# arielnetworks/tidal-wave

Hardware: AMD Instinct MI355X
Metric: image-pairs/sec @1080p Farneback (default params), 1/2/4/8 MI355X (higher is better)
Workload: dtype f32

## Files before the change

### tidal-wave_amd/csrc/twflow.hip

```cpp
#include "twflow_kernels.hip.h"

#include <hip/hip_runtime.h>
#include <unistd.h>

#include <dlfcn.h>
#include <float.h>
#include <math.h>
#include <stdio.h>
#include <stdlib.h>
#include <string.h>

#include <chrono>
#include <map>
#include <mutex>
#include <string>
#include <tuple>
#include <utility>
#include <vector>

#include "../../include/twflow.h"
#include "../../include/twflow_debug.h"

using namespace twk;

// ... 398 lines not shown
    int upd_ny = 2;
    int scan_fused = 0;
    int poly_f32 = 0;
    long long mfree_min_px = 0;
    int mfree_min_w = 320;
    int mfree = 1;
    int cu_count = 256;
    int pyr23_threads = 0;
    int blur_cm = 0;
    int pyr_fused = 1;
    int pyr_generic = 0;
    int blur_variant = 4;
    int pp_waves = 512;
    unsigned long long* dbg_stamps = nullptr;
    int blur_nomask = 0;
    int blur_pipe = 0;
    int blur_small = -1;
    int blur_small_lv[8] = {-1, -1, -1, -1, -1, -1, -1, -1};
    int poly_variant = 1;
    std::string err;
    size_t ws_elems = 0;
    float *I = nullptr, *R = nullptr, *M[2] = {nullptr, nullptr};
    std::vector<float*> flow;
    std::vector<size_t> flow_cap;
    int lat_streams = 1;
    long long lat_min_px = 100000;
    float *lat_I = nullptr, *lat_R = nullptr;
    size_t lat_cap = 0;
    std::vector<hipEvent_t> lat_ev;
    int lat_s2_max = 1000;
    int ramp = 1;
    int fi_maxseg = 4, fi_minsteps = 16;
    int fi_skip = 0;
    int fi_nt = 1024;
    int lat_fused = 1;
    int lat_graph = 0;
    std::map<GraphKey, hipGraphExec_t> lat_graphs;
    hipStream_t copy_stream = nullptr;
    hipStream_t d2h_stream = nullptr;
    long long d2h_ops = 0;
    int d2h_sync_skipped = 0;
    FlowDst* d_fdst = nullptr;
    FlowDst* d_fsrc = nullptr;
    const uint8_t** d_ptrs = nullptr;
    int* d_count = nullptr;
    float2* d_grid = nullptr;
    size_t d_grid_cap = 0;
    int prof_level[TW_K_COUNT] = {-2, -2, -2, -2, -2};
    std::vector<ProfPair> prof_pending[TW_K_COUNT];
    std::vector<hipEvent_t> prof_free;
    unsigned long long launches[TW_DF_COUNT] = {};
    unsigned long long last_grid_z[TW_DF_COUNT] = {};
};

namespace {

#define TW_LAUNCH(e, fam, kern, grid, ...)                         \
    do {                                                           \
        const dim3 _g = (grid);                                    \
        if (e) {                                                   \
            (e)->launches[fam]++;                                  \
            (e)->last_grid_z[fam] = _g.z;                          \
        }                                                          \
        hipLaunchKernelGGL(kern, _g, __VA_ARGS__);                 \
    } while (0)

#define TW_HIP(e, call)                                                                   \
// ... 635 lines not shown
    return pl->levels >= 1 && pl->lv[0].ksize == 3 && pl->lv[1].ksize == 3 && pl->lv[0].mode == 0 && pl->lv[1].mode == 2 &&
           pl->w0 == 2 * pl->lv[1].w && pl->h0 == 2 * pl->lv[1].h && pl->w0 >= 16;
}
void launch_pyr01(tw_engine* e, hipStream_t st, const Plan* pl, const uint8_t* const* d_srcs, long long stride, float* I1,
                  float* I0, int nimg)
{
    const LevelPlan &L0 = pl->lv[0], &L1 = pl->lv[1];
    PyrK3fArgs a;
    a.srcs = d_srcs;
    a.dst0 = I0;
    a.dst1 = I1;
    a.zs0 = L0.ps;
    a.zs1 = L1.ps;
    a.stride = stride;
    a.w0 = pl->w0;
    a.h0 = pl->h0;
    a.ld0 = L0.ld;
    a.w1 = L1.w;
    a.h1 = L1.h;
    a.ld1 = L1.ld;
    a.a0 = L0.h_kern[1];
    a.a1 = L0.h_kern[0];
    a.b0 = L1.h_kern[1];
    a.b1 = L1.h_kern[0];
    a.aligned4 = (stride % 4 == 0) ? e->img_aligned4 : 0;
    ProfScope ps(e, st, TW_K_PYR, 1);
    TW_LAUNCH(e, TW_DF_PYR_K3F, tw_pyr_k3f, dim3((L1.w + 255) / 256, (L1.h + 3) / 4, nimg), dim3(256), 0, st, a);
}

bool flow_iter_eligible(const tw_engine* e, int w, int h)
{
    return e->win_m == 15 && !e->box && w >= e->mfree_min_w && h >= 4 * FI_TH;
}
bool level_runs_flow_iter(const tw_engine* e, int w, int h, int nc, bool lat, bool grid_only)
{
    const int it = e->p.pyrIterations;
    const int fi_out = (e->fi_nt == 512 ? FI_SC_512 : FI_SC) - 30;
    const long long fi_wgs = (long long)((w + fi_out - 1) / fi_out) * std::min(4, std::max(1, h / (16 * FI_TH))) * nc;
    return e->mfree && !lat && it > (grid_only ? 1 : 0) && flow_iter_eligible(e, w, h) &&
           (fi_wgs * 4 >= (long long)e->cu_count * 3 || e->mfree == 2) &&
           (e->mfree_min_px <= 0 || (long long)w * h >= e->mfree_min_px);
}
bool single_pair_schedule(const tw_engine* e, int n, int w0, int h0, int levels)
{
    return n == 1 && e->lat_streams && levels >= 1 && (long long)w0 * h0 >= e->lat_min_px;
}
bool scan_fused_level0(const tw_engine* e, int span)
{
    return e->p.pyrIterations > 0 && e->scan_fused && span == 10 && e->win_m == 15 && !e->box;
}
int balanced_launch_pairs(int n, int chunk)
{
    const int nlaunch = (n + chunk - 1) / chunk;
    return nlaunch > 0 ? (n + nlaunch - 1) / nlaunch : 1;
}
struct FlowUps {
    const float* prev;
    int pw, ph, pld;
    long long pfps;
    const int *xofs, *yofs;
    const float *alpha, *beta;
    int xmax;
    float scale;
};
void launch_flow_iter(tw_engine* e, hipStream_t st, int w, int h, int ld, long long ps, const float* R, const float* flow_in,
                      long long fps_in, float* flow_out, long long fps_out, const FlowUps* ups, int npairs, int level)
{
    FlowIterArgs a;
    memset(&a, 0, sizeof(a));
    a.R = R;
    a.flow_in = flow_in;
    a.flow_out = flow_out;
    a.w = w;
    a.h = h;
    a.ld = ld;
    a.ps = ps;
    a.fps_in = fps_in;
    a.fps_out = fps_out;
    a.zero_flow = (!flow_in && !ups) ? 1 : 0;
    a.c = e->wc;
#ifdef TW_VARIANTS
    a.dbg_skip = e->fi_skip;
    a.dbg = (unsigned long long*)e->dbg_stamps;
#endif
    const int OUT = (e->fi_nt == 512 ? FI_SC_512 : FI_SC) - 30;
    const int slots = e->cu_count * (e->fi_nt == 512 ? 2 : 1);
    const int nstrips = (w + OUT - 1) / OUT, nsteps = (h + FI_TH - 1) / FI_TH;
    int best_seg = 1;
    double best_cost = 1e300;
    for (int sg = 1; sg <= e->fi_maxseg; sg++) {
        const int nt = (nsteps + sg - 1) / sg;
        if (sg > 1 && nt < e->fi_minsteps) break;
        const long long wgs = (long long)nstrips * sg * npairs;
        const long long rounds = (wgs + slots - 1) / slots;
        const double cost = (double)rounds * (nt + 7 * 0.25);
        if (cost < best_cost) {
            best_cost = cost;
            best_seg = sg;
        }
    }
    a.nt = (nsteps + best_seg - 1) / best_seg;
    const int nseg = (nsteps + a.nt - 1) / a.nt;
    const dim3 grid(nstrips, nseg, npairs);
    ProfScope pscope(e, st, TW_K_BLUR_SOLVE, level);
    if (ups) {
        a.prev = ups->prev;
        a.pw = ups->pw;
        a.ph = ups->ph;
        a.pld = ups->pld;
        a.pfps = ups->pfps;
        a.xofs = ups->xofs;
        a.alpha = ups->alpha;
        a.yofs = ups->yofs;
        a.beta = ups->beta;
        a.xmax = ups->xmax;
        a.scale = ups->scale;
    }
#ifdef TW_VARIANTS
    if (e->fi_nt == 512) {
        if (ups) TW_LAUNCH(e, TW_DF_FLOW_ITER_UPS, (tw_flow_iter<15, 1, 512>), grid, dim3(512), 0, st, a);
        else if (a.zero_flow) TW_LAUNCH(e, TW_DF_FLOW_ITER_ZERO, (tw_flow_iter<15, 2, 512>), grid, dim3(512), 0, st, a);
        else TW_LAUNCH(e, TW_DF_FLOW_ITER, (tw_flow_iter<15, 0, 512>), grid, dim3(512), 0, st, a);
        return;
    }
#endif
    if (ups) {
        TW_LAUNCH(e, TW_DF_FLOW_ITER_UPS, (tw_flow_iter<15, 1>), grid, dim3(1024), 0, st, a);
    } else if (a.zero_flow) {
        TW_LAUNCH(e, TW_DF_FLOW_ITER_ZERO, (tw_flow_iter<15, 2>), grid, dim3(1024), 0, st, a);
    } else {
        TW_LAUNCH(e, TW_DF_FLOW_ITER, (tw_flow_iter<15, 0>), grid, dim3(1024), 0, st, a);
    }
}

struct GridOut {
    float2* g;
    int span, gw, gh;
    bool* used;
};
void launch_blur(tw_engine* e, hipStream_t st, int w, int h, int ld, long long ps, const float* Min, float* Mout,
                 float* flow, const float* R, int update, int level, int npairs, double* Vbox = nullptr,
                 const SideJob* side = nullptr, bool* side_used = nullptr, const GridOut* go = nullptr, bool quads = false)
{
    BlurArgs a;
    a.Min = Min;
    a.Mout = Mout;
    a.flow = flow;
    a.R = R;
    a.w = w;
    a.h = h;
    a.ld = ld;
    a.ps = ps;
    a.fps = ps;
    a.update = update;
    a.xsh = 0;
    a.rot = 0;
    a.store_flow = level < 0 ? 1 : 0;
    a.m = e->win_m;
// ... 1381 lines not shown
            e->blur_small_lv[k] = atoi(q);
            while (*q && *q != ',') q++;
            if (*q == ',') q++;
        }
    }
    if (const char* ev = getenv("TW_PP_WAVES")) e->pp_waves = atoi(ev);
    if (const char* ev = getenv("TW_BLUR_NOMASK")) e->blur_nomask = atoi(ev);
    if (const char* ev = getenv("TW_BLUR_PIPE")) e->blur_pipe = atoi(ev);
    if (const char* ev = getenv("TW_POLYEXP_F32")) e->poly_f32 = atoi(ev) == 2 ? 2 : (atoi(ev) ? 1 : 0);
#ifndef TW_VARIANTS
    {
        bool bad_lv = false;
        for (int v : e->blur_small_lv) bad_lv = bad_lv || v == 2 || v == 3 || v == 5;
        const bool bad = bad_lv || (e->blur_variant != 4) || (e->poly_variant != 1) || (e->blur_pipe != 0) || (e->blur_small == 2 || e->blur_small == 3 ||
                         e->blur_small == 5) || (getenv("TW_UPD_NY") && atoi(getenv("TW_UPD_NY")) == 1);
        if (bad) {
            fprintf(stderr, "twflow: TW_BLUR_VARIANT / TW_POLY_VARIANT / TW_BLUR_PIPE / TW_BLUR_SMALL=2,3,5 / TW_UPD_NY=1 select kernels "
                            "that are only in a VARIANTS=1 build (tidal-wave_amd/libtwflow_variants.so)\n");
            delete e;
            return TW_E_UNSUPPORTED;
        }
    }
#endif
    if (const char* ev = getenv("TW_DEBUG_STAMPS"))
        if (atoi(ev) && hipMalloc((void**)&e->dbg_stamps, 4096 * sizeof(unsigned long long)) == hipSuccess)
            (void)hipMemset(e->dbg_stamps, 0, 4096 * sizeof(unsigned long long));
    if (const char* ev = getenv("TW_UPD_NY")) e->upd_ny = atoi(ev) == 1 ? 1 : 2;
    if (const char* ev = getenv("TW_LANES")) e->lanes = std::min(2, std::max(1, atoi(ev)));
    if (const char* ev = getenv("TW_LATENCY_STREAMS")) e->lat_streams = atoi(ev) ? 1 : 0;
    if (const char* ev = getenv("TW_LATENCY_MIN_PX")) e->lat_min_px = atoll(ev);
    if (const char* ev = getenv("TW_LAT_GRAPH")) e->lat_graph = atoi(ev) ? 1 : 0;
    if (const char* ev = getenv("TW_LAT_FUSED")) e->lat_fused = atoi(ev) ? 1 : 0;
#ifdef TW_VARIANTS
    if (const char* ev = getenv("TW_FI_NT")) e->fi_nt = atoi(ev) == 512 ? 512 : 1024;
    if (const char* ev = getenv("TW_FI_SKIP")) e->fi_skip = atoi(ev);
#endif
    if (const char* ev = getenv("TW_LAT_S2_LEVELS")) e->lat_s2_max = atoi(ev);
    if (const char* ev = getenv("TW_RAMP")) e->ramp = atoi(ev) ? 1 : 0;
    if (const char* ev = getenv("TW_FI_MAXSEG")) e->fi_maxseg = std::min(64, std::max(1, atoi(ev)));
    if (const char* ev = getenv("TW_FI_MINSTEPS")) e->fi_minsteps = std::max(2, atoi(ev));
    int prio_lo = 0, prio_hi = 0;
    (void)hipDeviceGetStreamPriorityRange(&prio_lo, &prio_hi);
    bool ok = hipStreamCreateWithPriority(&e->stream, hipStreamNonBlocking, prio_hi) == hipSuccess &&
              hipStreamCreateWithPriority(&e->stream2, hipStreamNonBlocking, e->lanes > 1 ? prio_hi : prio_lo) == hipSuccess &&
              hipStreamCreateWithFlags(&e->copy_stream, hipStreamNonBlocking) == hipSuccess &&
              hipEventCreateWithFlags(&e->ev_fork, hipEventDisableTiming) == hipSuccess &&
              hipEventCreateWithFlags(&e->ev_join, hipEventDisableTiming) == hipSuccess &&
              hipMalloc((void**)&e->d_ptrs, sizeof(void*) * 2 * slots + 256) == hipSuccess &&
              hipMalloc((void**)&e->d_count, sizeof(int) * slots + 256) == hipSuccess;
    for (Ctx& c : e->ctx) {
        ok = ok && hipEventCreate(&c.ev_start) == hipSuccess && hipEventCreate(&c.ev_stop) == hipSuccess &&
             hipEventCreateWithFlags(&c.ev_done, hipEventDisableTiming) == hipSuccess &&
             hipEventCreateWithFlags(&c.ev_h2d, hipEventDisableTiming) == hipSuccess &&
             hipEventCreateWithFlags(&c.ev_seg[0], hipEventDisableTiming) == hipSuccess &&
             hipEventCreateWithFlags(&c.ev_seg[1], hipEventDisableTiming) == hipSuccess &&
             hipHostMalloc((void**)&c.h_ptrs, sizeof(void*) * 2 * slots, hipHostMallocDefault) == hipSuccess &&
             hipHostMalloc((void**)&c.h_count, sizeof(int) * slots, hipHostMallocDefault) == hipSuccess &&
             hipHostMalloc((void**)&c.h_png, sizeof(PngJob) * 2 * (size_t)slots, hipHostMallocDefault) == hipSuccess &&
             hipMalloc((void**)&c.d_png, sizeof(PngJob) * 2 * (size_t)slots + 256) == hipSuccess &&
             hipHostMalloc((void**)&c.h_rec, sizeof(ScanRec) * HOST_RECS * (size_t)slots, hipHostMallocDefault) ==
                 hipSuccess;
    }
    if (!ok) {
        tw_engine_destroy(e);
        return TW_E_DEVICE;
    }
    *out = e;
// ... 1135 lines not shown
```

### tidal-wave_amd/csrc/twflow_kernels.hip.h

```cpp
#pragma once
#include <hip/hip_runtime.h>
#include <stdint.h>
#include <type_traits>

namespace twk {

typedef float __attribute__((ext_vector_type(4))) f32x4;
typedef const float __attribute__((address_space(1))) * gptr_cf;
typedef const char __attribute__((address_space(1))) * gptr_cc;

__device__ __forceinline__ gptr_cf sgpr_base(const float* p)
{
    gptr_cf g = (gptr_cf)p;
    asm volatile("" : "+s"(g));
    return g;
}
__device__ __forceinline__ float gload(gptr_cf row, unsigned byte_off)
{
    return *(gptr_cf)((gptr_cc)row + byte_off);
}
typedef float __attribute__((address_space(1))) * gptr_f;
typedef char __attribute__((address_space(1))) * gptr_c;
__device__ __forceinline__ gptr_f sgpr_base_w(float* p)
{
// ... 1795 lines not shown
            bstore(rsF, ob, 0u, fxv);
            bstore(rsF, ob, (unsigned)(a.fps * 4), fyv);
            if (a.gspan > 0) {
                const unsigned qx = __umulhi((unsigned)xc, a.gmagic), qy = __umulhi((unsigned)yc, a.gmagic);
                if (qx * (unsigned)a.gspan == (unsigned)xc && qy * (unsigned)a.gspan == (unsigned)yc)
                    a.grid[((long long)z * a.gh + qy) * a.gw + qx] = float2{fxv, fyv};
            }
        }
        if (FUSED) {
            if (a.update) {
                float M[5];
                if constexpr (QPRE) update_matrices_core(qpre[i], R1, a.ps, a.ld, a.w, a.h, xc, yc, fxv, fyv, M);
                else update_matrices_px(R0, R1, a.ps, a.ld, a.w, a.h, xc, yc, fxv, fyv, M);
                if (valid) {
                    if constexpr ((TW_NT & 1) == 0) {
#pragma unroll
                        for (int cc = 0; cc < 5; cc++) bstore(rsM, ob, (unsigned)(cc * a.ps * 4), M[cc]);
                    } else {
#pragma unroll
                        for (int cc = 0; cc < 5; cc++) st_stream<0>(Mout + o + cc * a.ps, M[cc]);
                    }
                }
            }
        }
    }
}
template <int MH, int COLS, int HALO, int TH, bool FUSED, int VILP = 2, int HILP = 2, int SUNROLL = 2, bool QPRE = true, bool VPRE = true>
__global__ __launch_bounds__(COLS) __attribute__((amdgpu_waves_per_eu(4, 8))) void tw_blur_solve4(BlurArgs a)
{
    __shared__ __attribute__((aligned(16))) float sm[5][TH][COLS];
    tw_blur_solve4_body<MH, COLS, HALO, TH, FUSED, VILP, HILP, SUNROLL, QPRE, VPRE>(a, hw_grid(), hw_block(), sm);
}

constexpr int FI_TH = 5, FI_SC = 190, FI_PITCH = 192;
constexpr int FI_SC_512 = 94, FI_PITCH_512 = 96;
struct FlowIterArgs {
    const float* R;
    const float* flow_in;
    float* flow_out;
    int w, h, ld;
    long long ps, fps_in, fps_out;
    int nt;
    int zero_flow;
    const float* prev;
    int pw, ph, pld;
    long long pfps;
    const int* xofs;
    const float* alpha;
    const int* yofs;
    const float* beta;
    int xmax;
    float scale;
    unsigned long long* dbg;
    int dbg_skip;
    WinCoef c;
};

#ifdef TW_VARIANTS
#define TW_FI_SKIP(bit) (a.dbg_skip & (bit))
#define TW_FI_SYNC() do { if (!TW_FI_SKIP(16)) __syncthreads(); } while (0)
#define TW_FI_STAMP(i)                                                                                                   \
    do {                                                                                                                 \
        if (a.dbg && (tid == 0 || tid == NT / 2 + 64) && fi_blin < 32 && st >= 40 && st < 48)                              \
            a.dbg[(((size_t)fi_blin * 2 + (tid ? 1 : 0)) * 8 + (st - 40)) * 8 + (i)] = __builtin_amdgcn_s_memtime();       \
    } while (0)
#else
#define TW_FI_SKIP(bit) false
#define TW_FI_SYNC() __syncthreads()
#define TW_FI_STAMP(i) do { } while (0)
#endif
template <int MH, int MODE, int NT = 1024>
__global__ __launch_bounds__(NT) __attribute__((amdgpu_waves_per_eu(4, 4))) void tw_flow_iter(FlowIterArgs a)
{
    constexpr bool UPS = MODE == 1;
#ifndef TW_FI_DEEP
#define TW_FI_DEEP 1
#endif
    constexpr bool DEEP = TW_FI_DEEP && MODE != 1 && NT == 1024;
#ifndef TW_FI_DIST
#define TW_FI_DIST 0
#endif
#define TW_FI_P(ph, sl) ((ph) * 8 + (sl))
    constexpr int DIST[4][10] = {
        {TW_FI_P(0, 0), TW_FI_P(0, 0), TW_FI_P(1, 0), TW_FI_P(1, 0), TW_FI_P(1, 1), TW_FI_P(1, 1), TW_FI_P(2, 0), TW_FI_P(2, 0), TW_FI_P(2, 0), TW_FI_P(2, 0)},
        {TW_FI_P(0, 1), TW_FI_P(0, 3), TW_FI_P(1, 0), TW_FI_P(1, 1), TW_FI_P(1, 2), TW_FI_P(1, 3), TW_FI_P(2, 0), TW_FI_P(2, 0), TW_FI_P(2, 1), TW_FI_P(2, 1)},
        {TW_FI_P(2, 0), TW_FI_P(2, 0), TW_FI_P(2, 0), TW_FI_P(2, 0), TW_FI_P(2, 0), TW_FI_P(2, 0), TW_FI_P(2, 0), TW_FI_P(2, 0), TW_FI_P(2, 0), TW_FI_P(2, 0)},
        {TW_FI_P(0, 0), TW_FI_P(0, 0), TW_FI_P(0, 1), TW_FI_P(0, 1), TW_FI_P(0, 2), TW_FI_P(0, 2), TW_FI_P(0, 3), TW_FI_P(0, 3), TW_FI_P(0, 4), TW_FI_P(0, 4)},
    };
    constexpr int TH = FI_TH, SC = NT == 1024 ? FI_SC : FI_SC_512, P = NT == 1024 ? FI_PITCH : FI_PITCH_512, OUT = SC - 2 * MH,
                  RING = TH + 2 * MH, NCH = RING / TH, NB = NCH + 1;
    static_assert(RING % TH == 0 && SC <= P && TH * SC <= NT && TH == 5 && OUT % 4 == 0 && 5 * TH * (OUT / 4) <= NT && (NB & (NB - 1)) == 0, "geometry");
    constexpr int VWAVES = (TH * SC + 63) / 64;
    constexpr bool SPLIT = VWAVES * 64 < NT;
    __shared__ __attribute__((aligned(16))) float blk[NB][5][TH][P];
    const int tid = threadIdx.x;
    int bx, seg, z;
    xcd_remap(bx, seg, z);
    const unsigned fi_blin = blockIdx.x + gridDim.x * (blockIdx.y + gridDim.y * blockIdx.z);
    (void)fi_blin;
    const WinCoef& c = a.c;
    const float* __restrict__ R0 = a.R + (long long)(2 * z) * 5 * a.ps;
    const float* __restrict__ R1 = R0 + 5 * a.ps;
    const float* __restrict__ fin = a.flow_in + (long long)z * 2 * a.fps_in;
    float* __restrict__ fout = a.flow_out + (long long)z * 2 * a.fps_out;
    const bool cth = tid < TH * SC;
    const int cr = cth ? tid / SC : 0, cc = cth ? tid - cr * SC : 0;
    const int xc = clampi(bx * OUT - MH + cc, 0, a.w - 1);
    const int ys = seg * a.nt * TH;
    const int nsteps = min(a.nt, (a.h - ys + TH - 1) / TH);
    if (nsteps <= 0) return;

    int sx = 0, sx1 = 0;
    bool two = false;
    float ua0 = 0.f, ua1 = 0.f;
    if (UPS) {
        sx = a.xofs[xc];
        sx1 = min(sx + 1, a.pw - 1);
        two = xc < a.xmax;
        ua0 = a.alpha[2 * xc];
        ua1 = a.alpha[2 * xc + 1];
    }
    const float* __restrict__ prev = UPS ? a.prev + (long long)z * 2 * a.pfps : nullptr;
// ... 61 lines not shown
    }
    unsigned go0 = 0, go1 = 0;
    unsigned gq = 0;
    auto gather_r0 = [&](int ch, float q[5]) { q[ch] = gload(r0b[ch], gq); };
    auto gather_head = [&](int k, float dx, float dy, float q[5], UpdTaps& T, bool with_r0) {
        const int yc = row_of(k);
        gq = (unsigned)(yc * a.ld + xc) * 4u;
        if (with_r0) {
#pragma unroll
            for (int ch = 0; ch < 5; ch++) gather_r0(ch, q);
        }
        const float fx = (float)xc + dx, fy = (float)yc + dy;
        const float flx = floorf(fx), fly = floorf(fy);
        const bool inb = flx >= 0.f && flx < (float)(a.w - 1) && fly >= 0.f && fly < (float)(a.h - 1);
        const int x1 = inb ? (int)flx : 0, y1 = inb ? (int)fly : 0;
        T.fx = fx - (float)x1;
        T.fy = fy - (float)y1;
        T.inb = inb;
        go0 = (unsigned)(y1 * a.ld + x1) * 4u;
        go1 = go0 + (unsigned)a.ld * 4u;
    };
    const __amdgpu_buffer_rsrc_t rs1 = make_rsrc(R1);
    unsigned r1off[5];
#pragma unroll
    for (int ch = 0; ch < 5; ch++) r1off[ch] = (unsigned)((long long)ch * a.ps * 4);
    auto gather_plane = [&](int ch, UpdTaps& T) {
        const f32x2 t01 = bload2(rs1, go0, r1off[ch]);
        const f32x2 t23 = bload2(rs1, go1, r1off[ch]);
        T.t[ch][0] = t01.x;
        T.t[ch][1] = t01.y;
        T.t[ch][2] = t23.x;
        T.t[ch][3] = t23.y;
    };
    auto gather_half = [&](int ch, int half, UpdTaps& T) {
        if (TW_FI_SKIP(32) && ch >= 3) return;
        const f32x2 t = bload2(rs1, half ? go1 : go0, r1off[ch]);
        T.t[ch][2 * half] = t.x;
        T.t[ch][2 * half + 1] = t.y;
    };
    auto gather_issue = [&](int k, float dx, float dy, float q[5], UpdTaps& T) {
        gather_head(k, dx, dy, q, T, true);
#pragma unroll
        for (int ch = 0; ch < 5; ch++) gather_plane(ch, T);
    };
    auto combine_store = [&](int k, float dx, float dy, const float q[5], const UpdTaps& T) {
        float M[5];
        update_matrices_combine(q, T, a.w, a.h, xc, row_of(k), dx, dy, M);
#pragma unroll
        for (int ch = 0; ch < 5; ch++) blk[k % NB][ch][cr][cc] = M[ch];
    };

    FlowIn fcur, fnext;
    float q[5];
    UpdTaps T;
    float dx = 0.f, dy = 0.f;
    UpdTaps Tb;
    float dxb = 0.f, dyb = 0.f;
    if (cth) {
        ytab_issue(0);
        flow_issue(0, fcur);
        ytab_issue(1);
#pragma unroll 1
        for (int k = 0; k < NCH; k++) {
            flow_issue(k + 1, fnext);
            ytab_issue(k + 2);
            flow_value(fcur, dx, dy);
            gather_issue(k, dx, dy, q, T);
            combine_store(k, dx, dy, q, T);
            fcur = fnext;
        }
        if constexpr (DEEP) {
            FlowIn f2;
            flow_issue(NCH + 1, f2);
            ytab_issue(NCH + 2);
            flow_value(fnext, dx, dy);
            gather_head(NCH, dx, dy, q, T, false);
#pragma unroll
            for (int ch = 0; ch < 5; ch++) gather_plane(ch, T);
            flow_value(f2, dxb, dyb);
            gather_head(NCH + 1, dxb, dyb, q, Tb, false);
        } else {
        flow_value(fnext, dx, dy);
        gather_head(NCH, dx, dy, q, T, true);
        }
    }
    __syncthreads();

    constexpr int NQ = OUT / 4;
    const bool hth = tid < 5 * TH * NQ;
    const int hp = hth ? tid / (TH * NQ) : 0, hrem = hth ? tid - hp * (TH * NQ) : 0, hr = hrem / NQ, hq = hrem - hr * NQ;
    constexpr int SMAIN = SPLIT ? (TH * OUT) / 64 * 64 : TH * OUT;
    const int sitem = tid < SMAIN ? tid : (SPLIT && tid >= VWAVES * 64 && tid - VWAVES * 64 < TH * OUT - SMAIN) ? SMAIN + tid - VWAVES * 64 : -1;
    const bool sth = sitem >= 0;
    const int sr = sth ? sitem / OUT : 0, sc = sth ? sitem - sr * OUT : 0;
    const int sxo = bx * OUT + sc;
    const __amdgpu_buffer_rsrc_t rso = make_rsrc(fout);
    const unsigned fout_p1 = (unsigned)(a.fps_out * 4);
    auto s_phase = [&](int st, int s0) {
        const int sy = ys + st * TH + sr;
        if (sth && sxo < a.w && sy < a.h && !TW_FI_SKIP(8)) {
            const double g11 = blk[s0][0][sr][sc], g12 = blk[s0][1][sr][sc], g22 = blk[s0][2][sr][sc],
                         h1 = blk[s0][3][sr][sc], h2 = blk[s0][4][sr][sc];
            const double idet = 1. / (g11 * g22 - g12 * g12 + 1e-3);
            const unsigned o = (unsigned)(sy * a.ld + sxo) * 4u;
            bstore(rso, o, 0u, (float)((g11 * h2 - g12 * h1) * idet));
            bstore(rso, o, fout_p1, (float)((g22 * h1 - g12 * h2) * idet));
        }
    };

    auto h_phase = [&](int s0, int bX, auto with_loads_c, UpdTaps& Tl) {
        constexpr bool WITH_LOADS = decltype(with_loads_c)::value;
        constexpr int HPLANE0 = DEEP ? 1 : 3;
        float v[4 + 2 * MH + 2];
        const f32x4* W4 = (const f32x4*)&blk[bX][hp][hr][4 * hq];
#pragma unroll
        for (int u = 0; u < (4 + 2 * MH + 2) / 4; u++) {
            const f32x4 t = W4[u];
            v[4 * u] = t[0];
            v[4 * u + 1] = t[1];
            v[4 * u + 2] = t[2];
            v[4 * u + 3] = t[3];
        }
        f32x4 o;
#pragma unroll
        for (int j = 0; j < 4; j++) {
            const int li = MH + j;
            float sum = v[li] * c.k[0];
#pragma unroll
            for (int i = 1; i <= MH; i++) sum += c.k[i] * (v[li - i] + v[li + i]);
            o[j] = sum;
            __builtin_amdgcn_sched_barrier(0);
            if constexpr (WITH_LOADS) {
                if constexpr (DEEP) {
#pragma unroll
                    for (int u = 0; u < 10; u++)
                        if (DIST[TW_FI_DIST][u] == TW_FI_P(1, j)) gather_half(u >> 1, u & 1, Tl);
                } else {
                    if (j < 2) gather_plane(HPLANE0 + j, Tl);
                }
            }
            __builtin_amdgcn_sched_barrier(0);
        }
        *(f32x4*)&blk[s0][hp][hr][4 * hq] = o;
    };

    if (SPLIT && tid >= VWAVES * 64) {
#pragma unroll 1
        for (int st = 0; st < nsteps; st++) {
            const int s0 = st & (NB - 1), bX = (st + NCH) & (NB - 1);
            TW_FI_SYNC();
            if (hth && !TW_FI_SKIP(4)) h_phase(s0, bX, std::false_type(), T);
            TW_FI_SYNC();
            s_phase(st, s0);
            TW_FI_SYNC();
        }
        return;
    }

    auto step = [&](int st, float (&qc)[5], float (&qn)[5]) {
        const bool more = st + 1 < nsteps;
        const int s0 = st & (NB - 1), bX = (st + NCH) & (NB - 1);
        TW_FI_STAMP(0);
        if (cth) {
            flow_issue(st + NCH + 1, fnext);
            ytab_issue(st + NCH + 2);
            gq = (unsigned)(row_of(st + NCH + 1) * a.ld + xc) * 4u;
            __builtin_amdgcn_sched_barrier(0);
            float wv[RING];
#pragma unroll
            for (int j = 0; j < NCH; j++) {
                const float* bj = &blk[(s0 + j) & (NB - 1)][cr][0][cc];
#pragma unroll
                for (int r = 0; r < TH; r++) wv[TH * j + r] = bj[r * P];
            }
            float* vout = &blk[bX][cr][0][cc];
#pragma unroll
            for (int r = 0; r < TH; r++) {
                float sv = wv[r + MH] * c.k[0];
#pragma unroll
                for (int i = 1; i <= MH; i++) sv += (wv[r + MH + i] + wv[r + MH - i]) * c.k[i];
                vout[r * P] = sv;
                __builtin_amdgcn_sched_barrier(0);
                if (r < 3) gather_plane(r, T);
                gather_r0(r, qn);
                __builtin_amdgcn_sched_barrier(0);
            }
        }
        TW_FI_STAMP(1);
        TW_FI_SYNC();
        TW_FI_STAMP(2);

        if (!TW_FI_SKIP(4)) h_phase(s0, bX, std::true_type(), T);
        TW_FI_STAMP(3);
        TW_FI_SYNC();
        TW_FI_STAMP(4);

        s_phase(st, s0);
        __builtin_amdgcn_sched_barrier(0);
        TW_FI_STAMP(5);
        if (cth) {
            if (more && !TW_FI_SKIP(1)) combine_store(st + NCH, dx, dy, qc, T);
            __builtin_amdgcn_sched_barrier(0);
            TW_FI_STAMP(6);
            flow_value(fnext, dx, dy);
            gather_head(st + NCH + 1, dx, dy, qn, T, false);
            __builtin_amdgcn_sched_barrier(0);
        }
        TW_FI_STAMP(7);
        TW_FI_SYNC();
    };
    auto step_deep = [&](int st, float& dxc, float& dyc, UpdTaps& Tc, float& dxn, float& dyn, UpdTaps& Tn) {
        const bool more = st + 1 < nsteps;
        const int s0 = st & (NB - 1), bX = (st + NCH) & (NB - 1);
        TW_FI_STAMP(0);
        if (cth) {
            flow_issue(st + NCH + 2, fnext);
            ytab_issue(st + NCH + 3);
            gq = (unsigned)(row_of(st + NCH) * a.ld + xc) * 4u;
            __builtin_amdgcn_sched_barrier(0);
            float wv[RING];
#pragma unroll
            for (int j = 0; j < NCH; j++) {
                const float* bj = &blk[(s0 + j) & (NB - 1)][cr][0][cc];
#pragma unroll
                for (int r = 0; r < TH; r++) wv[TH * j + r] = bj[r * P];
            }
            float* vout = &blk[bX][cr][0][cc];
#pragma unroll
            for (int r = 0; r < TH; r++) {
                float sv = wv[r + MH] * c.k[0];
#pragma unroll
                for (int i = 1; i <= MH; i++) sv += (wv[r + MH + i] + wv[r + MH - i]) * c.k[i];
                vout[r * P] = sv;
                __builtin_amdgcn_sched_barrier(0);
                gather_r0(r, q);
#pragma unroll
                for (int u = 0; u < 10; u++)
                    if (DIST[TW_FI_DIST][u] == TW_FI_P(0, r)) gather_half(u >> 1, u & 1, Tn);
                __builtin_amdgcn_sched_barrier(0);
            }
        }
        TW_FI_STAMP(1);
        TW_FI_SYNC();
        TW_FI_STAMP(2);
        if (!TW_FI_SKIP(4)) h_phase(s0, bX, std::true_type(), Tn);
        TW_FI_STAMP(3);
        TW_FI_SYNC();
        TW_FI_STAMP(4);
        s_phase(st, s0);
        __builtin_amdgcn_sched_barrier(0);
        TW_FI_STAMP(5);
        if (cth) {
#pragma unroll
            for (int u = 0; u < 10; u++)
                if (DIST[TW_FI_DIST][u] == TW_FI_P(2, 0)) gather_half(u >> 1, u & 1, Tn);
            __builtin_amdgcn_sched_barrier(0);
            if (more && !TW_FI_SKIP(1)) combine_store(st + NCH, dxc, dyc, q, Tc);
            __builtin_amdgcn_sched_barrier(0);
#pragma unroll
            for (int u = 0; u < 10; u++)
                if (DIST[TW_FI_DIST][u] == TW_FI_P(2, 1)) gather_half(u >> 1, u & 1, Tn);
            __builtin_amdgcn_sched_barrier(0);
            TW_FI_STAMP(6);
            flow_value(fnext, dxc, dyc);
            gather_head(st + NCH + 2, dxc, dyc, q, Tc, false);
            __builtin_amdgcn_sched_barrier(0);
        }
        TW_FI_STAMP(7);
        TW_FI_SYNC();
    };
    if constexpr (DEEP) {
        int st = 0;
#pragma unroll 1
        for (; st + 1 < nsteps; st += 2) {
            step_deep(st, dx, dy, T, dxb, dyb, Tb);
            step_deep(st + 1, dxb, dyb, Tb, dx, dy, T);
        }
        if (st < nsteps) step_deep(st, dx, dy, T, dxb, dyb, Tb);
        return;
    }
    float q1[5] = {0.f, 0.f, 0.f, 0.f, 0.f};
    {
        int st = 0;
#pragma unroll 1
        for (; st + 1 < nsteps; st += 2) {
            step(st, q, q1);
            step(st + 1, q1, q);
        }
        if (st < nsteps) step(st, q, q1);
    }
}

template <int MH, int COLS, int HALO, int TH, bool FUSED, int VILP = 2, int HILP = 2>
__global__ __launch_bounds__(COLS) __attribute__((amdgpu_waves_per_eu(4, 8))) void tw_blur_solve4q(BlurArgs a)
{
    constexpr int TW = COLS - 2 * HALO;
    constexpr int NW = TH + 2 * MH;
    __shared__ __attribute__((aligned(16))) float sm[5][TH][COLS];
    const int tid = threadIdx.x;
    int bx, by, z;
    xcd_remap(bx, by, z);
    const int x0 = bx * TW - a.xsh, y0 = by * TH;
    const WinCoef& c = a.c;
    const float* __restrict__ Min = a.Min + (long long)z * 5 * a.ps;
    float* __restrict__ flow = a.flow + (long long)z * 2 * a.fps;
    const int cx0 = max(0, -x0), vw = min(TW, a.w - x0) - cx0;
    const bool partial = !a.nomask && vw <= TW - 32;
    const int gq0 = cx0 >> 2, gv = ((cx0 + vw + 3) >> 2) - gq0;
    const float inv_gv = 1.f / (float)gv;

    if (a.nomask || (x0 - HALO + tid >= -MH && x0 - HALO + tid <= a.w - 1 + MH)) {
        const unsigned xb = (unsigned)clampi(x0 - HALO + tid, 0, a.w - 1) * 4u;
        unsigned ro[NW];
#pragma unroll
        for (int i = 0; i < NW; i++) ro[i] = (unsigned)clampi(y0 - MH + i, 0, a.h - 1) * ((unsigned)a.ld * 4u);
        float wa[NW], wb[NW];
        {
            const __amdgpu_buffer_rsrc_t rs = make_rsrc(Min);
#pragma unroll
            for (int i = 0; i < NW; i++) wa[i] = bload(rs, xb, ro[i]);
        }
#pragma unroll
        for (int ch = 0; ch < 5; ch++) {
// ... 1718 lines not shown
```

Measured before the change: 4746.

## Split flow-iteration kernel into producer/consumer wave roles for non-upsampling levels

Replaces the lockstep flow-iteration kernel for zero-flow and plain modes with a warp-specialized design. Four waves gather and combine matrices at raised priority while twelve waves run the vertical/horizontal blur and the solve, over a deeper ring buffer of blur blocks. The strip width narrows to fit the larger ring in LDS, and the upsampling mode keeps the old lockstep kernel without the deep variant. The 512-thread variant and the DEEP gather distribution are removed. The aim is to overlap gather latency with the blur math, at the cost of more halo overhead per strip and a role imbalance risk.

Measured after the change: 4698. 0.99x the previous value.

```diff
diff --git a/tidal-wave_amd/csrc/twflow.hip b/tidal-wave_amd/csrc/twflow.hip
--- a/tidal-wave_amd/csrc/twflow.hip
+++ b/tidal-wave_amd/csrc/twflow.hip
@@ -454,7 +454,6 @@
     int ramp = 1;
     int fi_maxseg = 4, fi_minsteps = 16;
     int fi_skip = 0;
-    int fi_nt = 1024;
     int lat_fused = 1;
     int lat_graph = 0;
     std::map<GraphKey, hipGraphExec_t> lat_graphs;
@@ -1156,11 +1155,11 @@
 {
     return e->win_m == 15 && !e->box && w >= e->mfree_min_w && h >= 4 * FI_TH;
 }
+constexpr int FI_GATE_COLS = 160;
 bool level_runs_flow_iter(const tw_engine* e, int w, int h, int nc, bool lat, bool grid_only)
 {
     const int it = e->p.pyrIterations;
-    const int fi_out = (e->fi_nt == 512 ? FI_SC_512 : FI_SC) - 30;
-    const long long fi_wgs = (long long)((w + fi_out - 1) / fi_out) * std::min(4, std::max(1, h / (16 * FI_TH))) * nc;
+    const long long fi_wgs = (long long)((w + FI_GATE_COLS - 1) / FI_GATE_COLS) * std::min(4, std::max(1, h / (16 * FI_TH))) * nc;
     return e->mfree && !lat && it > (grid_only ? 1 : 0) && flow_iter_eligible(e, w, h) &&
            (fi_wgs * 4 >= (long long)e->cu_count * 3 || e->mfree == 2) &&
            (e->mfree_min_px <= 0 || (long long)w * h >= e->mfree_min_px);
@@ -1207,8 +1206,8 @@
     a.dbg_skip = e->fi_skip;
     a.dbg = (unsigned long long*)e->dbg_stamps;
 #endif
-    const int OUT = (e->fi_nt == 512 ? FI_SC_512 : FI_SC) - 30;
-    const int slots = e->cu_count * (e->fi_nt == 512 ? 2 : 1);
+    const int OUT = ups ? FI_OUT_UPS : FI_OUT;
+    const int slots = e->cu_count;
     const int nstrips = (w + OUT - 1) / OUT, nsteps = (h + FI_TH - 1) / FI_TH;
     int best_seg = 1;
     double best_cost = 1e300;
@@ -1240,14 +1239,6 @@
         a.xmax = ups->xmax;
         a.scale = ups->scale;
     }
-#ifdef TW_VARIANTS
-    if (e->fi_nt == 512) {
-        if (ups) TW_LAUNCH(e, TW_DF_FLOW_ITER_UPS, (tw_flow_iter<15, 1, 512>), grid, dim3(512), 0, st, a);
-        else if (a.zero_flow) TW_LAUNCH(e, TW_DF_FLOW_ITER_ZERO, (tw_flow_iter<15, 2, 512>), grid, dim3(512), 0, st, a);
-        else TW_LAUNCH(e, TW_DF_FLOW_ITER, (tw_flow_iter<15, 0, 512>), grid, dim3(512), 0, st, a);
-        return;
-    }
-#endif
     if (ups) {
         TW_LAUNCH(e, TW_DF_FLOW_ITER_UPS, (tw_flow_iter<15, 1>), grid, dim3(1024), 0, st, a);
     } else if (a.zero_flow) {
@@ -2695,7 +2686,6 @@
     if (const char* ev = getenv("TW_LAT_GRAPH")) e->lat_graph = atoi(ev) ? 1 : 0;
     if (const char* ev = getenv("TW_LAT_FUSED")) e->lat_fused = atoi(ev) ? 1 : 0;
 #ifdef TW_VARIANTS
-    if (const char* ev = getenv("TW_FI_NT")) e->fi_nt = atoi(ev) == 512 ? 512 : 1024;
     if (const char* ev = getenv("TW_FI_SKIP")) e->fi_skip = atoi(ev);
 #endif
     if (const char* ev = getenv("TW_LAT_S2_LEVELS")) e->lat_s2_max = atoi(ev);
diff --git a/tidal-wave_amd/csrc/twflow_kernels.hip.h b/tidal-wave_amd/csrc/twflow_kernels.hip.h
--- a/tidal-wave_amd/csrc/twflow_kernels.hip.h
+++ b/tidal-wave_amd/csrc/twflow_kernels.hip.h
@@ -1851,8 +1851,8 @@
     tw_blur_solve4_body<MH, COLS, HALO, TH, FUSED, VILP, HILP, SUNROLL, QPRE, VPRE>(a, hw_grid(), hw_block(), sm);
 }
 
-constexpr int FI_TH = 5, FI_SC = 190, FI_PITCH = 192;
-constexpr int FI_SC_512 = 94, FI_PITCH_512 = 96;
+constexpr int FI_TH = 5, FI_SC = 150, FI_PITCH = 152, FI_MH = 15, FI_OUT = FI_SC - 2 * FI_MH;
+constexpr int FI_SC_UPS = 190, FI_PITCH_UPS = 192, FI_OUT_UPS = FI_SC_UPS - 2 * FI_MH;
 struct FlowIterArgs {
     const float* R;
     const float* flow_in;
@@ -1880,7 +1880,7 @@
 #define TW_FI_SYNC() do { if (!TW_FI_SKIP(16)) __syncthreads(); } while (0)
 #define TW_FI_STAMP(i)                                                                                                   \
     do {                                                                                                                 \
-        if (a.dbg && (tid == 0 || tid == NT / 2 + 64) && fi_blin < 32 && st >= 40 && st < 48)                              \
+        if (a.dbg && (tid == 0 || tid == NWIN) && fi_blin < 32 && st >= 40 && st < 48)                                    \
             a.dbg[(((size_t)fi_blin * 2 + (tid ? 1 : 0)) * 8 + (st - 40)) * 8 + (i)] = __builtin_amdgcn_s_memtime();       \
     } while (0)
 #else
@@ -1888,25 +1888,250 @@
 #define TW_FI_SYNC() __syncthreads()
 #define TW_FI_STAMP(i) do { } while (0)
 #endif
-template <int MH, int MODE, int NT = 1024>
-__global__ __launch_bounds__(NT) __attribute__((amdgpu_waves_per_eu(4, 4))) void tw_flow_iter(FlowIterArgs a)
-{
-    constexpr bool UPS = MODE == 1;
-#ifndef TW_FI_DEEP
-#define TW_FI_DEEP 1
-#endif
-    constexpr bool DEEP = TW_FI_DEEP && MODE != 1 && NT == 1024;
-#ifndef TW_FI_DIST
-#define TW_FI_DIST 0
-#endif
-#define TW_FI_P(ph, sl) ((ph) * 8 + (sl))
-    constexpr int DIST[4][10] = {
-        {TW_FI_P(0, 0), TW_FI_P(0, 0), TW_FI_P(1, 0), TW_FI_P(1, 0), TW_FI_P(1, 1), TW_FI_P(1, 1), TW_FI_P(2, 0), TW_FI_P(2, 0), TW_FI_P(2, 0), TW_FI_P(2, 0)},
-        {TW_FI_P(0, 1), TW_FI_P(0, 3), TW_FI_P(1, 0), TW_FI_P(1, 1), TW_FI_P(1, 2), TW_FI_P(1, 3), TW_FI_P(2, 0), TW_FI_P(2, 0), TW_FI_P(2, 1), TW_FI_P(2, 1)},
-        {TW_FI_P(2, 0), TW_FI_P(2, 0), TW_FI_P(2, 0), TW_FI_P(2, 0), TW_FI_P(2, 0), TW_FI_P(2, 0), TW_FI_P(2, 0), TW_FI_P(2, 0), TW_FI_P(2, 0), TW_FI_P(2, 0)},
-        {TW_FI_P(0, 0), TW_FI_P(0, 0), TW_FI_P(0, 1), TW_FI_P(0, 1), TW_FI_P(0, 2), TW_FI_P(0, 2), TW_FI_P(0, 3), TW_FI_P(0, 3), TW_FI_P(0, 4), TW_FI_P(0, 4)},
+template <int MH, int MODE, int NT>
+__device__ __forceinline__ void tw_flow_iter_roles(const FlowIterArgs& a)
+{
+    static_assert(MODE == 0 || MODE == 2, "the upsampling iteration runs tw_flow_iter_lockstep");
+    constexpr int TH = FI_TH, SC = FI_SC, P = FI_PITCH, OUT = SC - 2 * MH, RING = TH + 2 * MH, NCH = RING / TH, NB = NCH + 3;
+    constexpr int NWIN = NT - 256, NCL = NT - NWIN, NG = (TH * SC + NCL - 1) / NCL, NQ = OUT / 4;
+    static_assert(NT == 1024 && MH == FI_MH && RING % TH == 0 && TH == 5 && OUT % 4 == 0 && P % 4 == 0 && P >= SC + 2 &&
+                      4 * (NQ - 1) + 4 + 2 * MH + 2 <= P && 5 * SC <= NWIN && 5 * TH * NQ <= NWIN && TH * OUT <= NWIN &&
+                      NB * 5 * TH * P * 4 <= 160 * 1024,
+                  "geometry");
+    __shared__ __attribute__((aligned(16))) float blk[NB][5][TH][P];
+    const int tid = threadIdx.x;
+    int bx, seg, z;
+    xcd_remap(bx, seg, z);
+    const unsigned fi_blin = blockIdx.x + gridDim.x * (blockIdx.y + gridDim.y * blockIdx.z);
+    (void)fi_blin;
+    const WinCoef& c = a.c;
+    const int ys = seg * a.nt * TH;
+    const int nsteps = min(a.nt, (a.h - ys + TH - 1) / TH);
+    if (nsteps <= 0) return;
+    const int wave = __builtin_amdgcn_readfirstlane(tid >> 6);
+
+    if (wave >= NWIN / 64) {
+        const float* __restrict__ R0 = a.R + (long long)(2 * z) * 5 * a.ps;
+        const float* __restrict__ R1 = R0 + 5 * a.ps;
+        const int ctid = tid - NWIN;
+        __builtin_amdgcn_s_setprio(1);
+        struct Px {
+            int cr, cc, xc;
+        };
+        auto act = [&](int g) { return g * NCL + ctid < TH * SC; };
+        auto px_of = [&](int g) {
+            const int l = ctid;
+            Px p;
+            p.cr = min(g * NCL + l, TH * SC - 1) / SC;
+            p.cc = min(g * NCL + l, TH * SC - 1) - p.cr * SC;
+            p.xc = clampi(bx * OUT - MH + p.cc, 0, a.w - 1);
+            return p;
+        };
+        auto row_of = [&](int k, const Px& p) { return clampi(ys - MH + TH * k + p.cr, 0, a.h - 1); };
+        struct FlowIn {
+            float p[2];
+        };
+        const float* __restrict__ fin = a.flow_in + (long long)z * 2 * a.fps_in;
+        const __amdgpu_buffer_rsrc_t rsf = make_rsrc(MODE == 0 ? (const void*)fin : (const void*)R0);
+        const unsigned fin_p1 = (unsigned)(a.fps_in * 4);
+        auto flow_issue = [&](int k, int g, FlowIn& f) {
+            if constexpr (MODE == 2) {
+                f.p[0] = f.p[1] = 0.f;
+            } else {
+                const Px p = px_of(g);
+                const unsigned o = (unsigned)(row_of(k, p) * a.ld + p.xc) * 4u;
+                f.p[0] = bload(rsf, o, 0u);
+                f.p[1] = bload(rsf, o, fin_p1);
+            }
+        };
+        auto flow_value = [&](const FlowIn& f, float& dx, float& dy) {
+            asm volatile("v_mov_b32 %0, %2\n\tv_mov_b32 %1, %3" : "=&v"(dx), "=&v"(dy) : "v"(f.p[0]), "v"(f.p[1]));
+        };
+        gptr_cf r0b[5];
+#pragma unroll
+        for (int ch = 0; ch < 5; ch++) r0b[ch] = sgpr_base(R0 + ch * a.ps);
+        const __amdgpu_buffer_rsrc_t rs1 = make_rsrc(R1);
+        unsigned r1off[5];
+#pragma unroll
+        for (int ch = 0; ch < 5; ch++) r1off[ch] = (unsigned)((long long)ch * a.ps * 4);
+        auto gather_head = [&](int k, const Px& p, float dx, float dy, UpdTaps& T, int& x1, int& y1) {
+            const int yc = row_of(k, p);
+            const float fx = (float)p.xc + dx, fy = (float)yc + dy;
+            const float flx = floorf(fx), fly = floorf(fy);
+            const bool inb = flx >= 0.f && flx < (float)(a.w - 1) && fly >= 0.f && fly < (float)(a.h - 1);
+            x1 = inb ? (int)flx : 0;
+            y1 = inb ? (int)fly : 0;
+            T.fx = fx - (float)x1;
+            T.fy = fy - (float)y1;
+            T.inb = inb;
+        };
+        auto gather_issue = [&](int k, const Px& p, float dx, float dy, float q[5], float (&t)[5][4]) {
+            const unsigned gq = (unsigned)(row_of(k, p) * a.ld + p.xc) * 4u;
+#pragma unroll
+            for (int ch = 0; ch < 5; ch++) q[ch] = gload(r0b[ch], gq);
+            UpdTaps H;
+            int x1, y1;
+            gather_head(k, p, dx, dy, H, x1, y1);
+            const unsigned go0 = (unsigned)(y1 * a.ld + x1) * 4u, go1 = go0 + (unsigned)a.ld * 4u;
+#pragma unroll
+            for (int ch = 0; ch < 5; ch++) {
+                const f32x2 t01 = bload2(rs1, go0, r1off[ch]);
+                const f32x2 t23 = bload2(rs1, go1, r1off[ch]);
+                t[ch][0] = t01.x;
+                t[ch][1] = t01.y;
+                t[ch][2] = t23.x;
+                t[ch][3] = t23.y;
+            }
+        };
+        static_assert(NG == 3, "one item per barrier interval");
+        float t[NG][5][4], q[NG][5], dx[NG], dy[NG];
+        FlowIn F[NG];
+        auto item = [&](int k, int cb, auto gc, bool combine) {
+            constexpr int g = decltype(gc)::value;
+            const Px p = px_of(g);
+            if (combine && !TW_FI_SKIP(1)) {
+                float M[5];
+                UpdTaps T;
+                int x1, y1;
+                gather_head(k, p, dx[g], dy[g], T, x1, y1);
+#pragma unroll
+                for (int ch = 0; ch < 5; ch++)
+#pragma unroll
+                    for (int u = 0; u < 4; u++) T.t[ch][u] = t[g][ch][u];
+                update_matrices_combine(q[g], T, a.w, a.h, p.xc, row_of(k, p), dx[g], dy[g], M);
+                if (act(g)) {
+#pragma unroll
+                    for (int ch = 0; ch < 5; ch++) blk[cb][ch][p.cr][p.cc] = M[ch];
+                }
+            }
+            __builtin_amdgcn_sched_barrier(0);
+            flow_value(F[g], dx[g], dy[g]);
+            flow_issue(k + 2, g, F[g]);
+            __builtin_amdgcn_sched_barrier(0);
+            gather_issue(k + 1, p, dx[g], dy[g], q[g], t[g]);
+            __builtin_amdgcn_sched_barrier(0);
+        };
+        using I0 = std::integral_constant<int, 0>;
+        using I1 = std::integral_constant<int, 1>;
+        using I2 = std::integral_constant<int, 2>;
+#pragma unroll
+        for (int g = 0; g < NG; g++) flow_issue(0, g, F[g]);
+        item(-1, 0, I0(), false);
+        item(-1, 0, I1(), false);
+        item(-1, 0, I2(), false);
+#pragma unroll 1
+        for (int k = 0; k < NCH; k++) {
+            item(k, k, I0(), true);
+            item(k, k, I1(), true);
+            item(k, k, I2(), true);
+        }
+        __syncthreads();
+        int cb = NCH;
+#pragma unroll 1
+        for (int st = 0; st < nsteps; st++) {
+            TW_FI_STAMP(0);
+            item(st + NCH, cb, I0(), true);
+            TW_FI_STAMP(1);
+            item(st + NCH, cb, I1(), true);
+            TW_FI_STAMP(2);
+            TW_FI_SYNC();
+            TW_FI_STAMP(3);
+            item(st + NCH, cb, I2(), true);
+            TW_FI_STAMP(4);
+            TW_FI_STAMP(7);
+            TW_FI_SYNC();
+            cb = cb + 1 == NB ? 0 : cb + 1;
+        }
+        return;
+    }
+
+    float* __restrict__ fout = a.flow_out + (long long)z * 2 * a.fps_out;
+    const bool vth = tid < 5 * SC;
+    const int vp = vth ? tid / SC : 0, vc = vth ? tid - vp * SC : 0;
+    const bool hth = tid < 5 * TH * NQ;
+    const int hp = hth ? tid / (TH * NQ) : 0, hrem = hth ? tid - hp * (TH * NQ) : 0, hr = hrem / NQ, hq = hrem - hr * NQ;
+    const bool sth = tid < TH * OUT;
+    const int sr = sth ? tid / OUT : 0, sc = sth ? tid - sr * OUT : 0;
+    const int sxo = bx * OUT + sc;
+    const __amdgpu_buffer_rsrc_t rso = make_rsrc(fout);
+    const unsigned fout_p1 = (unsigned)(a.fps_out * 4);
+    auto s_phase = [&](int st, int sY) {
+        const int sy = ys + st * TH + sr;
+        if (sth && sxo < a.w && sy < a.h && !TW_FI_SKIP(8)) {
+            const double g11 = blk[sY][0][sr][sc], g12 = blk[sY][1][sr][sc], g22 = blk[sY][2][sr][sc],
+                         h1 = blk[sY][3][sr][sc], h2 = blk[sY][4][sr][sc];
+            const double idet = 1. / (g11 * g22 - g12 * g12 + 1e-3);
+            const unsigned o = (unsigned)(sy * a.ld + sxo) * 4u;
+            bstore(rso, o, 0u, (float)((g11 * h2 - g12 * h1) * idet));
+            bstore(rso, o, fout_p1, (float)((g22 * h1 - g12 * h2) * idet));
+        }
     };
-    constexpr int TH = FI_TH, SC = NT == 1024 ? FI_SC : FI_SC_512, P = NT == 1024 ? FI_PITCH : FI_PITCH_512, OUT = SC - 2 * MH,
+    __syncthreads();
+    int s0 = 0;
+#pragma unroll 1
+    for (int st = 0; st < nsteps; st++) {
+        const int bX = s0 + NCH + 1 >= NB ? s0 + NCH + 1 - NB : s0 + NCH + 1;
+        TW_FI_STAMP(0);
+        if (st > 0) s_phase(st - 1, s0 == 0 ? NB - 1 : s0 - 1);
+        TW_FI_STAMP(1);
+        if (vth) {
+            float wv[RING];
+#pragma unroll
+            for (int j = 0; j < NCH; j++) {
+                const int b = s0 + j >= NB ? s0 + j - NB : s0 + j;
+                const float* bj = &blk[b][vp][0][vc];
+#pragma unroll
+                for (int r = 0; r < TH; r++) wv[TH * j + r] = bj[r * P];
+            }
+            float* vout = &blk[bX][vp][0][vc];
+#pragma unroll
+            for (int r = 0; r < TH; r++) {
+                float sv = wv[r + MH] * c.k[0];
+#pragma unroll
+                for (int i = 1; i <= MH; i++) sv += (wv[r + MH + i] + wv[r + MH - i]) * c.k[i];
+                vout[r * P] = sv;
+            }
+        }
+        TW_FI_STAMP(2);
+        TW_FI_SYNC();
+        TW_FI_STAMP(3);
+        if (hth && !TW_FI_SKIP(4)) {
+            float v[4 + 2 * MH + 2];
+            const f32x4* W4 = (const f32x4*)&blk[bX][hp][hr][4 * hq];
+#pragma unroll
+            for (int u = 0; u < (4 + 2 * MH + 2) / 4; u++) {
+                const f32x4 t = W4[u];
+                v[4 * u] = t[0];
+                v[4 * u + 1] = t[1];
+                v[4 * u + 2] = t[2];
+                v[4 * u + 3] = t[3];
+            }
+            f32x4 o;
+#pragma unroll
+            for (int j = 0; j < 4; j++) {
+                const int li = MH + j;
+                float sum = v[li] * c.k[0];
+#pragma unroll
+                for (int i = 1; i <= MH; i++) sum += c.k[i] * (v[li - i] + v[li + i]);
+                o[j] = sum;
+            }
+            *(f32x4*)&blk[s0][hp][hr][4 * hq] = o;
+        }
+        TW_FI_STAMP(4);
+        TW_FI_STAMP(7);
+        TW_FI_SYNC();
+        s0 = s0 + 1 == NB ? 0 : s0 + 1;
+    }
+    s_phase(nsteps - 1, s0 == 0 ? NB - 1 : s0 - 1);
+}
+
+template <int MH, int NT>
+__device__ __forceinline__ void tw_flow_iter_lockstep(const FlowIterArgs& a)
+{
+    constexpr int MODE = 1;
+    constexpr bool UPS = true, DEEP = false;
+    (void)DEEP;
+    constexpr int TH = FI_TH, SC = FI_SC_UPS, P = FI_PITCH_UPS, OUT = SC - 2 * MH,
                   RING = TH + 2 * MH, NCH = RING / TH, NB = NCH + 1;
     static_assert(RING % TH == 0 && SC <= P && TH * SC <= NT && TH == 5 && OUT % 4 == 0 && 5 * TH * (OUT / 4) <= NT && (NB & (NB - 1)) == 0, "geometry");
     constexpr int VWAVES = (TH * SC + 63) / 64;
@@ -2034,12 +2259,6 @@
         T.t[ch][2] = t23.x;
         T.t[ch][3] = t23.y;
     };
-    auto gather_half = [&](int ch, int half, UpdTaps& T) {
-        if (TW_FI_SKIP(32) && ch >= 3) return;
-        const f32x2 t = bload2(rs1, half ? go1 : go0, r1off[ch]);
-        T.t[ch][2 * half] = t.x;
-        T.t[ch][2 * half + 1] = t.y;
-    };
     auto gather_issue = [&](int k, float dx, float dy, float q[5], UpdTaps& T) {
         gather_head(k, dx, dy, q, T, true);
 #pragma unroll
@@ -2056,8 +2275,6 @@
     float q[5];
     UpdTaps T;
     float dx = 0.f, dy = 0.f;
-    UpdTaps Tb;
-    float dxb = 0.f, dyb = 0.f;
     if (cth) {
         ytab_issue(0);
         flow_issue(0, fcur);
@@ -2071,20 +2288,8 @@
             combine_store(k, dx, dy, q, T);
             fcur = fnext;
         }
-        if constexpr (DEEP) {
-            FlowIn f2;
-            flow_issue(NCH + 1, f2);
-            ytab_issue(NCH + 2);
-            flow_value(fnext, dx, dy);
-            gather_head(NCH, dx, dy, q, T, false);
-#pragma unroll
-            for (int ch = 0; ch < 5; ch++) gather_plane(ch, T);
-            flow_value(f2, dxb, dyb);
-            gather_head(NCH + 1, dxb, dyb, q, Tb, false);
-        } else {
         flow_value(fnext, dx, dy);
         gather_head(NCH, dx, dy, q, T, true);
-        }
     }
     __syncthreads();
 
@@ -2112,7 +2317,7 @@
 
     auto h_phase = [&](int s0, int bX, auto with_loads_c, UpdTaps& Tl) {
         constexpr bool WITH_LOADS = decltype(with_loads_c)::value;
-        constexpr int HPLANE0 = DEEP ? 1 : 3;
+        constexpr int HPLANE0 = 3;
         float v[4 + 2 * MH + 2];
         const f32x4* W4 = (const f32x4*)&blk[bX][hp][hr][4 * hq];
 #pragma unroll
@@ -2133,13 +2338,7 @@
             o[j] = sum;
             __builtin_amdgcn_sched_barrier(0);
             if constexpr (WITH_LOADS) {
-                if constexpr (DEEP) {
-#pragma unroll
-                    for (int u = 0; u < 10; u++)
-                        if (DIST[TW_FI_DIST][u] == TW_FI_P(1, j)) gather_half(u >> 1, u & 1, Tl);
-                } else {
-                    if (j < 2) gather_plane(HPLANE0 + j, Tl);
-                }
+                if (j < 2) gather_plane(HPLANE0 + j, Tl);
             }
             __builtin_amdgcn_sched_barrier(0);
         }
@@ -2162,7 +2361,6 @@
     auto step = [&](int st, float (&qc)[5], float (&qn)[5]) {
         const bool more = st + 1 < nsteps;
         const int s0 = st & (NB - 1), bX = (st + NCH) & (NB - 1);
-        TW_FI_STAMP(0);
         if (cth) {
             flow_issue(st + NCH + 1, fnext);
             ytab_issue(st + NCH + 2);
@@ -2188,99 +2386,22 @@
                 __builtin_amdgcn_sched_barrier(0);
             }
         }
-        TW_FI_STAMP(1);
         TW_FI_SYNC();
-        TW_FI_STAMP(2);
 
         if (!TW_FI_SKIP(4)) h_phase(s0, bX, std::true_type(), T);
-        TW_FI_STAMP(3);
         TW_FI_SYNC();
-        TW_FI_STAMP(4);
 
         s_phase(st, s0);
         __builtin_amdgcn_sched_barrier(0);
-        TW_FI_STAMP(5);
         if (cth) {
             if (more && !TW_FI_SKIP(1)) combine_store(st + NCH, dx, dy, qc, T);
             __builtin_amdgcn_sched_barrier(0);
-            TW_FI_STAMP(6);
             flow_value(fnext, dx, dy);
             gather_head(st + NCH + 1, dx, dy, qn, T, false);
             __builtin_amdgcn_sched_barrier(0);
         }
-        TW_FI_STAMP(7);
         TW_FI_SYNC();
     };
-    auto step_deep = [&](int st, float& dxc, float& dyc, UpdTaps& Tc, float& dxn, float& dyn, UpdTaps& Tn) {
-        const bool more = st + 1 < nsteps;
-        const int s0 = st & (NB - 1), bX = (st + NCH) & (NB - 1);
-        TW_FI_STAMP(0);
-        if (cth) {
-            flow_issue(st + NCH + 2, fnext);
-            ytab_issue(st + NCH + 3);
-            gq = (unsigned)(row_of(st + NCH) * a.ld + xc) * 4u;
-            __builtin_amdgcn_sched_barrier(0);
-            float wv[RING];
-#pragma unroll
-            for (int j = 0; j < NCH; j++) {
-                const float* bj = &blk[(s0 + j) & (NB - 1)][cr][0][cc];
-#pragma unroll
-                for (int r = 0; r < TH; r++) wv[TH * j + r] = bj[r * P];
-            }
-            float* vout = &blk[bX][cr][0][cc];
-#pragma unroll
-            for (int r = 0; r < TH; r++) {
-                float sv = wv[r + MH] * c.k[0];
-#pragma unroll
-                for (int i = 1; i <= MH; i++) sv += (wv[r + MH + i] + wv[r + MH - i]) * c.k[i];
-                vout[r * P] = sv;
-                __builtin_amdgcn_sched_barrier(0);
-                gather_r0(r, q);
-#pragma unroll
-                for (int u = 0; u < 10; u++)
-                    if (DIST[TW_FI_DIST][u] == TW_FI_P(0, r)) gather_half(u >> 1, u & 1, Tn);
-                __builtin_amdgcn_sched_barrier(0);
-            }
-        }
-        TW_FI_STAMP(1);
-        TW_FI_SYNC();
-        TW_FI_STAMP(2);
-        if (!TW_FI_SKIP(4)) h_phase(s0, bX, std::true_type(), Tn);
-        TW_FI_STAMP(3);
-        TW_FI_SYNC();
-        TW_FI_STAMP(4);
-        s_phase(st, s0);
-        __builtin_amdgcn_sched_barrier(0);
-        TW_FI_STAMP(5);
-        if (cth) {
-#pragma unroll
-            for (int u = 0; u < 10; u++)
-                if (DIST[TW_FI_DIST][u] == TW_FI_P(2, 0)) gather_half(u >> 1, u & 1, Tn);
-            __builtin_amdgcn_sched_barrier(0);
-            if (more && !TW_FI_SKIP(1)) combine_store(st + NCH, dxc, dyc, q, Tc);
-            __builtin_amdgcn_sched_barrier(0);
-#pragma unroll
-            for (int u = 0; u < 10; u++)
-                if (DIST[TW_FI_DIST][u] == TW_FI_P(2, 1)) gather_half(u >> 1, u & 1, Tn);
-            __builtin_amdgcn_sched_barrier(0);
-            TW_FI_STAMP(6);
-            flow_value(fnext, dxc, dyc);
-            gather_head(st + NCH + 2, dxc, dyc, q, Tc, false);
-            __builtin_amdgcn_sched_barrier(0);
-        }
-        TW_FI_STAMP(7);
-        TW_FI_SYNC();
-    };
-    if constexpr (DEEP) {
-        int st = 0;
-#pragma unroll 1
-        for (; st + 1 < nsteps; st += 2) {
-            step_deep(st, dx, dy, T, dxb, dyb, Tb);
-            step_deep(st + 1, dxb, dyb, Tb, dx, dy, T);
-        }
-        if (st < nsteps) step_deep(st, dx, dy, T, dxb, dyb, Tb);
-        return;
-    }
     float q1[5] = {0.f, 0.f, 0.f, 0.f, 0.f};
     {
         int st = 0;
@@ -2291,6 +2412,13 @@
         }
         if (st < nsteps) step(st, q, q1);
     }
+}
+
+template <int MH, int MODE, int NT = 1024>
+__global__ __launch_bounds__(NT) __attribute__((amdgpu_waves_per_eu(4, 4))) void tw_flow_iter(FlowIterArgs a)
+{
+    if constexpr (MODE == 1) tw_flow_iter_lockstep<MH, NT>(a);
+    else tw_flow_iter_roles<MH, MODE, NT>(a);
 }
 
 template <int MH, int COLS, int HALO, int TH, bool FUSED, int VILP = 2, int HILP = 2>
```
